# hello-robot/stretch_mujoco

Measured on AMD Instinct MI355X. Metric: env-steps/sec (whole node), 4096 parallel Stretch envs in total, higher is better.
Workload: dtype f32

## Files before the change

__graft_entry__.py:

```python
import os
import subprocess
import sys

ROOT = os.path.dirname(os.path.abspath(__file__))
sys.path.insert(0, ROOT)


def build() -> None:
    env = dict(os.environ)
    subprocess.check_call(["make", "-j6", "-C", os.path.join(ROOT, "stretch_mujoco_amd", "csrc")], env=env)
    subprocess.check_call(["make", "-C", os.path.join(ROOT, "oracle")], env=env)
    subprocess.check_call(["make", "-j4", "-C", os.path.join(ROOT, "tests", "emul")], env=env)
    subprocess.check_call(["make", "-j2", "-C", os.path.join(ROOT, "tests", "emul_contacts")], env=env)
    subprocess.check_call(["make", "-C", os.path.join(ROOT, "tests", "rccl_stub")], env=env)
    import stretch_mujoco_amd
    from stretch_mujoco_amd import lib

    L = lib.load()
    for sym in lib.EXPORTS:
        getattr(L, sym)


def smoke() -> None:
    import numpy as np
    import torch

    from oracle.oracle import Oracle
    from stretch_mujoco_amd import StretchBatchSimulator

    B, settle, nsteps = 8, 300, 100
    ctrl = np.array([2, -1, 0.6, 0.1, 1, -0.4, 0.5, 0.02, 0.3, -0.2], np.float32)
    o = Oracle(open(os.path.join(ROOT, "stretch_mujoco_amd", "models", "stretch_empty.smjb"), "rb").read())
    o.set_option("solver", 2)
    o.arr("ctrl")[:] = ctrl
    o.step(settle)
    sim = StretchBatchSimulator(num_envs=B, device="cuda:0", solver="newton")
    sim.start(home=False)
    dev = sim.device
    sim.ctrl[:] = torch.tensor(ctrl, device=dev).unsqueeze(1)
    sim.qpos[:] = torch.tensor(o.arr("qpos"), dtype=torch.float32, device=dev).unsqueeze(1)
    sim.qvel[:] = torch.tensor(o.arr("qvel"), dtype=torch.float32, device=dev).unsqueeze(1)
    sim.qacc_warmstart[:] = torch.tensor(o.arr("qacc_warmstart"), dtype=torch.float32, device=dev).unsqueeze(1)
    sim.step(nsteps)
    torch.cuda.synchronize()
    o.step(nsteps)
    qpos = sim.qpos.t().cpu().numpy()
    err = np.abs(qpos - o.arr("qpos")[None, :]).max()
    f = sim.info[3]
    flags = int(((f & 1).max() | (f & 2).max() | (f & 4).max() | (f & 8).max()).item())
    print(f"smoke: {B} envs x {nsteps} steps, max |qpos - oracle| = {err:.3e}, nefc = {int(sim.info[0, 0])}, flags = {flags}")
    assert np.isfinite(qpos).all(), "non-finite state"
    assert err < 1e-4, f"HIP path deviates from the fp64 oracle: {err}"
    assert flags == 0 and int(sim.nstep.min()) == int(sim.nstep.max()) == nsteps, "an env was flagged or ran fewer steps than asked"
    sim.stop()
    print(mujoco_status())


def mujoco_status() -> str:
    sys.path.insert(0, os.path.join(ROOT, "tools"))
    import mujoco_harness

    if not mujoco_harness.have_mujoco():
        return mujoco_harness.UNVERIFIED
    try:
        res = mujoco_harness.compare("stretch_empty", steps=1000)
        return res["verdict"] + " (tools/mujoco_harness.py; the HIP kernels are tested against that restatement)"
    except Exception as e:
        return f"mujoco is importable but the Appendix-D harness failed ({type(e).__name__}: {e}); MuJoCo parity UNVERIFIED"


if __name__ == "__main__":
    build()
    if len(sys.argv) > 1 and sys.argv[1] == "smoke":
        smoke()
```

stretch_mujoco_amd/csrc/smj_model.h:

```cpp
#pragma once
#include <stdint.h>

#if defined(SMJ_SAT)
#define NSAT SMJ_SAT
#define NVP 32
#ifndef SMJ_SAT_ROWS
#define SMJ_SAT_ROWS 320
#define SMJ_SAT_CONTACTS 64
#define SMJ_SAT_DENSE 256
#endif
#define NEFC SMJ_SAT_ROWS
#define NCON SMJ_SAT_CONTACTS
#define NDR SMJ_SAT_DENSE
#ifndef SMJ_SAT_EXT
#define SMJ_SAT_EXT 4
#endif
#ifndef SMJ_SAT_PGS
#define SMJ_SAT_PGS (SMJ_SAT_DENSE < 160 ? SMJ_SAT_DENSE : 160)
#endif
#define NXS SMJ_SAT_EXT
static_assert(NDR % 16 == 0 && NDR <= NEFC, "dense rows: whole 16-row blocks (matT_J, MFMA k-steps)");
#define NENT 5
#elif defined(SMJ_BIG)
#define NVP 64
#ifndef SMJ_NVS
#define SMJ_NVS 64
#endif
#define NVS SMJ_NVS
#if SMJ_NVS == 64
#define NEFC 224
#define NCON 64
#elif defined(SMJ_BIG_ROWS)
#define NEFC SMJ_BIG_ROWS
#define NCON SMJ_BIG_CONTACTS
#else
#define NEFC 160
#define NCON 48
#endif
#define NENT 8
#elif defined(SMJ_TALL)
#define NVP 32
#ifdef SMJ_TALL_ROWS
#define NEFC SMJ_TALL_ROWS
#define NCON SMJ_TALL_CONTACTS
#else
#define NEFC 160
#define NCON 48
#endif
#define NENT 5
#else
#define NVP 32
#define NEFC 80
#define NCON 16
#define NENT 5
#endif
#ifndef NVS
#define NVS NVP
#endif
#ifndef NSAT
#define NSAT 0
#endif
#ifndef NDR
#define NDR NEFC
#endif
static_assert(NVS % 2 == 0 && NVS <= NVP && (NVP == 64 ? NVS >= 38 : NVS == NVP), "column capacity: even (packed pairs), odd row stride NVS + 1");
#define NBP 32
#define NBT (NBP + NSAT)
#define NCG 128

#define SMJ_MODEL_I32(X)                                                                                          \
  X(body_parentid) X(k_body_jump) X(body_rootid) X(body_jntadr) X(body_jntnum) X(body_dofadr) X(body_dofnum) X(k_body_level)     \
  X(k_body_subtreesize) X(k_body_dofmask_lo) X(k_body_dofmask_hi) X(k_root_list) X(k_gc_body)                     \
  X(jnt_type) X(jnt_qposadr) X(jnt_dofadr) X(jnt_bodyid) X(jnt_limited)                                           \
  X(dof_bodyid) X(dof_jntid) X(dof_parentid) X(k_dof_anc_adr) X(k_dof_anc_num) X(k_dof_anc) X(k_dof_velmask_lo)   \
  X(k_dof_velmask_hi) X(k_dof_qposadr) X(k_ldl_i) X(k_ldl_j) X(k_ldl_lact) X(k_fric_dof) X(k_limit_jnt) X(k_act_dof) X(k_dof_act)                         \
  X(geom_type) X(geom_bodyid) X(geom_hulladr) X(geom_hullnum)                                                     \
  X(site_bodyid)                                                                           \
  X(eq_obj1id) X(eq_obj2id) X(eq_active)                                                                          \
  X(actuator_trntype) X(actuator_trnid) X(actuator_ctrllimited) X(actuator_forcelimited) X(actuator_biastype)     \
  X(pair_geom1) X(pair_geom2) X(pair_condim) X(k_planepair) X(k_cgeom) X(k_convpair) X(k_convpair_s1) X(k_convpair_s2) X(k_convpair_ss)

#define SMJ_MODEL_F32(X)                                                                                          \
  X(body_pos) X(body_quat) X(k_body_inertia_local) X(body_gcmass) X(body_gcipos) X(body_subtreemass)              \
  X(jnt_pos) X(jnt_axis) X(jnt_stiffness) X(jnt_range) X(jnt_margin) X(jnt_solref) X(jnt_solimp) X(qpos0)         \
  X(qpos_spring)                                                                                                  \
  X(dof_armature) X(dof_damping) X(dof_frictionloss) X(dof_invweight0) X(dof_solref) X(dof_solimp)                \
  X(geom_pos) X(k_geom_mat) X(geom_size) X(geom_rbound) X(k_geom_bcenter) X(geom_rgba) X(geom_invweight0)         \
  X(k_hull_vert4) X(geom_aabb) X(geom_ccenter) X(k_convpair_rsum) X(k_cgeom_half) X(k_cgeom_lcen)                                                                             \
  X(site_pos) X(k_site_mat)                                                                                       \
  X(eq_data) X(eq_solref) X(eq_solimp)                                                                            \
  X(actuator_gear) X(actuator_gainprm) X(actuator_biasprm) X(actuator_ctrlrange) X(actuator_forcerange)           \
  X(k_act_moment) X(key_ctrl) X(k_ldl_damp) X(k_ldl_dcoef) X(k_ldl_lcoef) X(k_act_mom) X(k_dof_actmom)                                                                                     \
  X(pair_friction) X(pair_solref) X(pair_solimp) X(pair_margin) X(pair_gap)

struct DevModel {
  int nq, nv, nu, nbody, njnt, ngeom, nsite, neq, npair, nlevel, nfric, nlimit, nplanepair, nldl, nlidar, imu_site,
      ngc, nroot, nkey, ncgeom, nconvpair, njump, maxsubtree;
  int iterations, warmstart, pgs_fixed_iter, max_con_pair, solver , ls_iterations, convex_pairs;
  float grad_noise;
  int pgs_island_stop;
  int qcqp_exact;
  int pgs_dual_ws;
  int sep_cache;
  int manifold_cache;
  int multi_serial;
  int pgs_cap;
  int row_limit;
  int multiccd;
  float ls_tolerance;
  float timestep, gravity[3], impratio, tolerance, meaninertia, lidar_cutoff;
  int nsat, nq_all, nv_all, nbody_all, nfric_main, nlimit_main;
  const int* k_satrec;
  int nsgeom, nstatpair, grid_dim[3];
  float grid_org[3], grid_h, grid_margin;
  const int* k_sgrec;
  const int* k_sprec;
  const int* k_spair;
  const int* k_grid_adr;
  const int* k_grid_list;
  const int* k_sg_cell;
  const float* k_sg_bound;
  const float* k_sgw;
#define X(n) const int* n;
  SMJ_MODEL_I32(X)
#undef X
#define X(n) const float* n;
  SMJ_MODEL_F32(X)
#undef X
  const int* k_lanerec;
  const int* k_pprec;
  const int* k_cgrec;
  const int* k_rowrec;
  const int* k_cprec;
};
enum { SMJ_CP_PAIR = 0, SMJ_CP_G1, SMJ_CP_G2, SMJ_CP_S1, SMJ_CP_S2, SMJ_CP_MARGIN, SMJ_CP_MG, SMJ_CP_CONDIM, SMJ_CP_FRIC = 8, SMJ_CP_SOLIMP = 13,
       SMJ_CP_SOLREF = 18, SMJ_CP_RBMIN = 20 ,
       SMJ_CP_B1 = 21, SMJ_CP_B2 = 22 , SMJ_CP_STRIDE = 24 };
enum { SMJ_RR_TYPE = 0, SMJ_RR_ID, SMJ_RR_D1, SMJ_RR_D2, SMJ_RR_Q1, SMJ_RR_Q2, SMJ_RR_V1, SMJ_RR_V2, SMJ_RR_DATA = 8, SMJ_RR_DIAG = 13,
       SMJ_RR_FLOSS = 14, SMJ_RR_SOLREF = 15, SMJ_RR_SOLIMP = 17, SMJ_RR_SAT = 22 , SMJ_RR_SDOF = 23 , SMJ_RR_STRIDE = 24 };
constexpr int smj_lr_act(int nent) { return 76 + ((7 * nent + 3) & ~3); }
constexpr int smj_lr_stride(int nent) { return smj_lr_act(nent) + 28; }
enum { SMJ_LR_KIN = 0, SMJ_LR_BODY = 36, SMJ_LR_DOF = 60, SMJ_LR_ENT = 76, SMJ_LR_ACT = smj_lr_act(NENT), SMJ_LR_STRIDE = smj_lr_stride(NENT) };
enum { SMJ_PP_PAIR = 0, SMJ_PP_G1, SMJ_PP_G2, SMJ_PP_B1, SMJ_PP_B2, SMJ_PP_T2, SMJ_PP_MARGIN, SMJ_PP_RBOUND2, SMJ_PP_BCEN2 = 8,
       SMJ_PP_POS1 = 11, SMJ_PP_MAT1 = 14, SMJ_PP_POS2 = 23, SMJ_PP_MAT2 = 26, SMJ_PP_SIZE2 = 35, SMJ_PP_CONDIM = 38, SMJ_PP_MG = 39,
       SMJ_PP_FRIC = 40, SMJ_PP_SOLIMP = 45, SMJ_PP_SOLREF = 50, SMJ_PP_BOX2 = 52 ,
       SMJ_PP_STRIDE = 60 };
enum { SMJ_CG_GEOM = 0, SMJ_CG_BODY, SMJ_CG_META, SMJ_CG_POS = 3, SMJ_CG_MAT = 6, SMJ_CG_LCEN = 15, SMJ_CG_HALF = 18, SMJ_CG_CCEN = 21,
       SMJ_CG_SIZE = 24, SMJ_CG_RBOUND = 27, SMJ_CG_STRIDE = 28 };

enum { SMJ_SR_BODY = 0, SMJ_SR_JTYPE, SMJ_SR_QADR, SMJ_SR_DADR, SMJ_SR_NDOF, SMJ_SR_JNT, SMJ_SR_F = 8,
       SMJ_SR_POS = SMJ_SR_F + 0, SMJ_SR_QUAT = SMJ_SR_F + 3, SMJ_SR_JPOS = SMJ_SR_F + 7, SMJ_SR_JAXIS = SMJ_SR_F + 10, SMJ_SR_Q0 = SMJ_SR_F + 13,
       SMJ_SR_INL = SMJ_SR_F + 14, SMJ_SR_ARM = SMJ_SR_F + 24, SMJ_SR_DAMP = SMJ_SR_F + 30, SMJ_SR_STIFF = SMJ_SR_F + 36, SMJ_SR_SPRING = SMJ_SR_F + 37,
       SMJ_SR_GCMASS = SMJ_SR_F + 38, SMJ_SR_GCIPOS = SMJ_SR_F + 39, SMJ_SR_STRIDE = 52 };
struct SmjStageLayout {
  int qpos, qvel, warm, ctrl, bctl, nstep, info, actlen, actvel, base, gyro, accel, xpose, stride;
};
constexpr SmjStageLayout smj_stage_layout(int nvp, int nbp, int nsat = 0) {
  SmjStageLayout L{};
  L.qpos = 0; L.qvel = L.qpos + nvp + 8 + 7 * nsat; L.warm = L.qvel + nvp + 6 * nsat; L.ctrl = L.warm + nvp + 6 * nsat; L.bctl = L.ctrl + 16; L.nstep = L.bctl + 8;
  L.info = L.nstep + 4; L.actlen = L.info + 4; L.actvel = L.actlen + 16; L.base = L.actvel + 16; L.gyro = L.base + 4;
  L.accel = L.gyro + 4; L.xpose = L.accel + 4; L.stride = L.xpose + 12 * nbp;
  return L;
}
struct DevState {
  int B;
  long ld;
  float* qpos;
  float* qvel;
  float* ctrl;
  float* warm;
  int* nstep;
  float* act_len;
  float* act_vel;
  float* base;
  float* gyro;
  float* accel;
  float* lidar;
  int* info;
  float* debug;
  float* prof;
  float* xpose;
  float* bctl;
  float* stage;
  SmjStageLayout lay;
  const int* order;
  int* cost;
  int* redo;
  int redo_worker;
// ... 68 lines not shown
```

stretch_mujoco_amd/csrc/smj_model_load.h:

```cpp
#pragma once
#include <stdint.h>
#include <stdio.h>
#include <math.h>
#include <string.h>

#include <map>
#include <string>
#include <vector>

#include "smj_model.h"

struct SmjBlobEntry {
  char name[48];
  uint32_t dtype, ndim, shape[4];
  uint64_t offset, nbytes;
};

struct SmjBlob {
  const uint8_t* p;
  size_t n;
  bool valid() const {
    if (!p || n < 16) return false;
    uint32_t cnt;
    memcpy(&cnt, p + 8, 4);
// ... 177 lines not shown
    int* k = rec.data() + (size_t)(nstat + L) * SMJ_RR_STRIDE;
    const int j = gi("k_limit_jnt", L >> 1), d = gi("jnt_dofadr", j);
    k[SMJ_RR_SAT] = sat_of(d, &k[SMJ_RR_SDOF]);
    k[SMJ_RR_TYPE] = 3; k[SMJ_RR_ID] = j; k[SMJ_RR_D1] = d; k[SMJ_RR_D2] = (L & 1) ? 1 : -1; k[SMJ_RR_Q1] = gi("jnt_qposadr", j);
    k[SMJ_RR_V1] = fb(gf("jnt_range", 2 * j + (L & 1))); k[SMJ_RR_V2] = fb(gf("jnt_margin", j));
    k[SMJ_RR_DIAG] = fb(gf("dof_invweight0", d));
    k[SMJ_RR_SOLREF] = fb(gf("jnt_solref", 2 * j)); k[SMJ_RR_SOLREF + 1] = fb(gf("jnt_solref", 2 * j + 1));
    for (int q = 0; q < 5; q++) k[SMJ_RR_SOLIMP + q] = fb(gf("jnt_solimp", 5 * j + q));
  }
  return rec;
}

static inline std::vector<int> smj_build_cprec(const DevModel& m, std::map<std::string, std::vector<int>>& I,
                                               std::map<std::string, std::vector<float>>& F, bool stat = false) {
  const int np = stat ? m.nstatpair : m.nconvpair;
  std::vector<int> rec((size_t)(np > 0 ? np : 1) * SMJ_CP_STRIDE, 0);
  auto fb = [](float v) { int b; memcpy(&b, &v, 4); return b; };
  auto gi = [&](const char* nm, size_t k) { const std::vector<int>& v = I[nm]; return k < v.size() ? v[k] : 0; };
  auto gf = [&](const char* nm, size_t k) { const std::vector<float>& v = F[nm]; return k < v.size() ? v[k] : 0.f; };
  std::map<int, int> dslot, sslot;
  if (stat) {
    for (int c = 0; c < m.ncgeom; c++) dslot[gi("k_cgeom", c)] = c;
    for (int c = 0; c < m.nsgeom; c++) sslot[gi("k_sgeom", c)] = c;
  }
  for (int t = 0; t < np; t++) {
    int* k = rec.data() + (size_t)t * SMJ_CP_STRIDE;
    const int p = gi(stat ? "k_statpair" : "k_convpair", t);
    k[SMJ_CP_PAIR] = p; k[SMJ_CP_G1] = gi("pair_geom1", p); k[SMJ_CP_G2] = gi("pair_geom2", p);
    if (stat) {
      k[SMJ_CP_S1] = sslot.count(k[SMJ_CP_G1]) ? -1 - sslot[k[SMJ_CP_G1]] : dslot[k[SMJ_CP_G1]];
      k[SMJ_CP_S2] = sslot.count(k[SMJ_CP_G2]) ? -1 - sslot[k[SMJ_CP_G2]] : dslot[k[SMJ_CP_G2]];
    } else { k[SMJ_CP_S1] = gi("k_convpair_s1", t); k[SMJ_CP_S2] = gi("k_convpair_s2", t); }
    k[SMJ_CP_MARGIN] = fb(gf("pair_margin", p)); k[SMJ_CP_MG] = fb(gf("pair_margin", p) - gf("pair_gap", p)); k[SMJ_CP_CONDIM] = gi("pair_condim", p);
    for (int q = 0; q < 5; q++) { k[SMJ_CP_FRIC + q] = fb(gf("pair_friction", 5 * p + q)); k[SMJ_CP_SOLIMP + q] = fb(gf("pair_solimp", 5 * p + q)); }
    k[SMJ_CP_SOLREF] = fb(gf("pair_solref", 2 * p)); k[SMJ_CP_SOLREF + 1] = fb(gf("pair_solref", 2 * p + 1));
    const float r1 = gf("geom_rbound", k[SMJ_CP_G1]), r2 = gf("geom_rbound", k[SMJ_CP_G2]);
    k[SMJ_CP_RBMIN] = fb(r1 < r2 ? r1 : r2);
    k[SMJ_CP_B1] = gi("geom_bodyid", k[SMJ_CP_G1]); k[SMJ_CP_B2] = gi("geom_bodyid", k[SMJ_CP_G2]);
  }
  return rec;
}

template <class Up>
int smj_load_model(const void* blob, size_t nbytes, DevModel& m, Up& up, std::string& err, const SmjCaps* caps, int ncaps, int* chosen) {
  if (!blob || nbytes < 16 || memcmp(blob, "SMJB0001", 8) != 0) { err = "not an SMJB model blob"; return -1; }
  SmjBlob b{static_cast<const uint8_t*>(blob), nbytes};
  if (!b.valid()) { err = "model blob: truncated or corrupt entry table"; return -3; }
  auto geti = [&](const char* name, int idx, int* out) -> bool {
    const SmjBlobEntry* e = b.find(name);
    if (!e || e->dtype != 1 || e->nbytes < 4u * (idx + 1)) { err = std::string("model blob: missing int ") + name; return false; }
    memcpy(out, b.p + e->offset + 4 * idx, 4);
    return true;
  };
  auto getf = [&](const char* name, int idx, float* out) -> bool {
    const SmjBlobEntry* e = b.find(name);
    if (!e || e->dtype != 0 || e->nbytes < 8u * (idx + 1)) { err = std::string("model blob: missing scalar ") + name; return false; }
    double v;
    memcpy(&v, b.p + e->offset + 8 * idx, 8);
    *out = (float)v;
    return true;
  };
#define GI(field, name, idx) if (!geti(name, idx, &m.field)) return -3;
#define GF(field, name, idx) if (!getf(name, idx, &m.field)) return -3;
  GI(nq_all, "dims", 0) GI(nv_all, "dims", 1) GI(nu, "dims", 2) GI(nbody_all, "dims", 3) GI(njnt, "dims", 4) GI(ngeom, "dims", 5)
  m.nq = m.nq_all; m.nv = m.nv_all; m.nbody = m.nbody_all; m.nsat = 0;
  if (b.find("k_nsat")) {
    GI(nsat, "k_nsat", 0)
    if (m.nsat > 0) { GI(nq, "k_main_dims", 0) GI(nv, "k_main_dims", 1) GI(nbody, "k_main_dims", 2) GI(njnt, "k_main_dims", 3) }
  }
  GI(nsite, "dims", 6) GI(neq, "dims", 8) GI(nkey, "dims", 11) GI(npair, "dims", 12)
  GI(nlevel, "k_nlevel", 0) GI(nfric, "k_nfric", 0) GI(nlimit, "k_nlimit", 0) GI(nplanepair, "k_nplanepair", 0)
  GI(nldl, "k_nldl", 0) GI(imu_site, "sensor_imu_site", 0) GI(ngc, "k_ngc", 0) GI(nroot, "k_nroot", 0)
  GI(njump, "k_njump", 0) GI(maxsubtree, "k_maxsubtree", 0) GI(ncgeom, "k_ncgeom", 0) GI(nconvpair, "k_nconvpair", 0) GI(iterations, "opt_iterations", 0)
  GF(timestep, "opt_timestep", 0) GF(gravity[0], "opt_gravity", 0) GF(gravity[1], "opt_gravity", 1)
  GF(gravity[2], "opt_gravity", 2) GF(impratio, "opt_impratio", 0) GF(tolerance, "opt_tolerance", 0)
  GF(meaninertia, "stat_meaninertia", 0) GF(lidar_cutoff, "sensor_lidar_cutoff", 0)
#undef GI
#undef GF
  if (m.nsat > 0 && (m.ngeom >= 65536 || m.npair >= (1 << 19))) { err = "satellite builds: at most 65535 geoms and 524287 collision pairs (16-bit geom ids per contact, the PGS row key)"; return -4; }
  {
    const SmjBlobEntry* e = b.find("sensor_lidar_site");
    m.nlidar = e ? (int)(e->nbytes / 4) : 0;
  }
  m.row_limit = 0; m.pgs_cap = 0; m.warmstart = 1; m.pgs_fixed_iter = 0; m.qcqp_exact = 0; m.grad_noise = 4e-6f; m.pgs_island_stop = 1; m.pgs_dual_ws = 1; m.max_con_pair = 4; m.solver = 0; m.convex_pairs = 1; m.multiccd = 1; m.sep_cache = getenv("SMJ_NO_SEPCACHE") ? 0 : 1; m.manifold_cache = (getenv("SMJ_NO_MCACHE") || m.nv_all <= 32) ? 0 : 1;    m.multi_serial = 0; m.ls_iterations = 50; m.ls_tolerance = 0.01f;
  char buf[256];
  int pick = -1, first = 0;
  {
    const SmjBlobEntry* e = b.find("k_capacity_hint");
    int hint = 0;
    if (e && e->dtype == 1 && e->nbytes >= 4) memcpy(&hint, b.p + e->offset, 4);
    if (hint > 0 && ncaps > 1) first = 1;
  }
  for (int v = first; v < ncaps && pick < 0; v++)
    if ((m.nsat > 0) == (caps[v].nsat > 0) && m.nsat <= caps[v].nsat &&
        m.nv <= (caps[v].nvs ? caps[v].nvs : caps[v].nvp) && m.nbody <= caps[v].nbp && m.nq <= caps[v].nvp + 8 && m.nldl <= caps[v].nent * 64) pick = v;
  if (pick < 0 && first > 0)
    for (int v = 0; v < first && pick < 0; v++)
      if ((m.nsat > 0) == (caps[v].nsat > 0) && m.nsat <= caps[v].nsat &&
          m.nv <= (caps[v].nvs ? caps[v].nvs : caps[v].nvp) && m.nbody <= caps[v].nbp && m.nq <= caps[v].nvp + 8 && m.nldl <= caps[v].nent * 64) pick = v;
  if (pick < 0 || m.nu > 16) {
    const SmjCaps& c = caps[ncaps - 1];
    snprintf(buf, sizeof buf, "model exceeds kernel capacity (nv %d<=%d, nbody %d<=%d, nq %d<=%d, nu %d<=16, mass-matrix entries %d<=%d, satellites %d)",
             m.nv, c.nvp, m.nbody, c.nbp, m.nq, c.nvp + 8, m.nu, m.nldl, c.nent * 64, m.nsat);
    err = buf;
    return -4;
  }
  if (chosen) *chosen = pick;
  const int nent = caps[pick].nent;
  if (m.neq + m.nfric > 64) { err = "too many static constraint rows"; return -4; }
  if (2 * m.nlimit > 64) { err = "too many limited joints"; return -4; }
  if (m.ngc > 16) { err = "more than 16 gravity-compensated bodies"; return -4; }
  if (m.njump > 6) { err = "body tree deeper than 64 levels"; return -4; }
  if (m.ncgeom > NCG) { err = "too many geoms in non-plane collision pairs"; return -4; }
  if (m.nconvpair >= 65536) { err = "more than 65535 non-plane collision pairs (the survivor list holds 16-bit pair indices)"; return -4; }
  std::map<std::string, std::vector<int>> hosti;
  std::map<std::string, std::vector<float>> hostf;
#define X(n)                                                                               \
  {                                                                                        \
    const SmjBlobEntry* e = b.find(#n);                                                    \
    if (!e || e->dtype != 1) { err = "model blob: missing i32 array " #n; return -3; }     \
    std::vector<int> h(e->nbytes / 4 ? e->nbytes / 4 : 1, 0);                              \
    memcpy(h.data(), b.p + e->offset, e->nbytes);                                          \
    m.n = up.i32(h);                                                                       \
    hosti[#n] = h;                                                                         \
    if (!m.n) { err = "device allocation failed for " #n; return -2; }                     \
  }
  SMJ_MODEL_I32(X)
#undef X
#define X(n)                                                                               \
  {                                                                                        \
    const SmjBlobEntry* e = b.find(#n);                                                    \
    if (!e || e->dtype != 0) { err = "model blob: missing f64 array " #n; return -3; }     \
    size_t cnt = e->nbytes / 8;                                                            \
    std::vector<float> h(cnt ? cnt : 1, 0.f);                                              \
    const double* src = reinterpret_cast<const double*>(b.p + e->offset);                  \
    for (size_t i = 0; i < cnt; i++) h[i] = (float)src[i];                                 \
    m.n = up.f32(h);                                                                       \
    hostf[#n] = h;                                                                         \
    if (!m.n) { err = "device allocation failed for " #n; return -2; }                     \
  }
  SMJ_MODEL_F32(X)
#undef X
  m.nsgeom = 0; m.nstatpair = 0; m.k_sgrec = m.k_sprec = m.k_spair = m.k_grid_adr = m.k_grid_list = m.k_sg_cell = nullptr; m.k_sg_bound = nullptr; m.k_sgw = nullptr;
  if (b.find("k_nsgeom")) {
    if (!geti("k_nsgeom", 0, &m.nsgeom) || !geti("k_nstatpair", 0, &m.nstatpair)) return -3;
    if (m.nsgeom > 512) { err = "more than 512 static collision geoms (the static broadphase's candidate word holds 9 bits of static geom index)"; return -4; }
    if (m.nstatpair > 0 && m.nsat == 0) { err = "static collision pairs (k_statpair) without satellites: only the satellite builds run collision_static; rebuild the blob (model_fuse.prepare_for_kernels)"; return -4; }
    if (m.nsgeom > 0) {
      for (int q = 0; q < 3; q++) { if (!geti("k_grid", q, &m.grid_dim[q]) || !getf("k_grid_f", q, &m.grid_org[q])) return -3; }
      if (!getf("k_grid_f", 3, &m.grid_h) || !getf("k_grid_f", 4, &m.grid_margin)) return -3;
      auto loadi = [&](const char* name, const int** dst) -> bool {
        const SmjBlobEntry* e = b.find(name);
        if (!e || e->dtype != 1) { err = std::string("model blob: missing i32 array ") + name; return false; }
        std::vector<int> h(e->nbytes / 4 ? e->nbytes / 4 : 1, 0);
        memcpy(h.data(), b.p + e->offset, e->nbytes);
        hosti[name] = h;
        *dst = up.i32(h);
        return *dst != nullptr;
      };
      const int* dummy = nullptr;
      if (!loadi("k_sgeom", &dummy) || !loadi("k_statpair", &dummy) || !loadi("k_spair", &m.k_spair) || !loadi("k_grid_adr", &m.k_grid_adr) ||
          !loadi("k_grid_list", &m.k_grid_list) || !loadi("k_sg_cell", &m.k_sg_cell)) return err.empty() ? -2 : -3;
      {
        const SmjBlobEntry* e = b.find("geom_aabb");
        (void)e;
      }
      std::vector<int> sg = smj_build_cgrec(m, hosti, hostf, true), spr = smj_build_cprec(m, hosti, hostf, true);
// ... 75 lines not shown
```

stretch_mujoco_amd/csrc/smj_step_impl.h:

```cpp
#pragma once
#ifndef SMJ_PROFILING
#define SMJ_PROFILING 1
#endif
#include <cstddef>
#include "smj_model.h"
#include "smj_wave.h"
#include "smj_sat_mem.h"

#define JS (NVS + 1)
#define MS (NVS + 1)
#define SMJ_MINVAL 1e-15f
#define SMJ_MINIMP 0.0001f
#define SMJ_MAXIMP 0.9999f

enum { JT_FREE = 0, JT_BALL = 1, JT_SLIDE = 2, JT_HINGE = 3 };
enum { GT_PLANE = 0, GT_SPHERE = 2, GT_CAPSULE = 3, GT_ELLIPSOID = 4, GT_CYLINDER = 5, GT_BOX = 6, GT_MESH = 7 };
enum { CT_EQUALITY = 0, CT_FRICTION = 1, CT_LIMIT = 3, CT_CONTACT_FRICTIONLESS = 5, CT_CONTACT_ELLIPTIC = 7, CT_NONE = -1 };

#if NSAT > 0
#define NCGS (NCG + 1)
#define NSURV 128
#else
#define NCGS NCG
#endif
// ... 181 lines not shown
      }
    }
    if (bad) {
#pragma unroll
      for (int i = 0; i < N; i++) res[i] = 0;
      return 0;
    }
    float x[N], nn = 0;
#pragma unroll
    for (int i = 0; i < N; i++) {
      float sv = -b[i];
#pragma unroll
      for (int k = 0; k < i; k++) sv -= L[i * N + k] * x[k];
      x[i] = sv * Li[i];
    }
#pragma unroll
    for (int i = N - 1; i >= 0; i--) {
      float sv = x[i];
#pragma unroll
      for (int k = i + 1; k < N; k++) sv -= L[k * N + i] * x[k];
      x[i] = sv * Li[i];
    }
#pragma unroll
    for (int i = 0; i < N; i++) { res[i] = x[i]; nn += x[i] * x[i]; }
    const float val = nn - r2;
    if (val < vtol && (exact || la == 0.f || val > -vtol)) break;
    float q = 0;
#pragma unroll
    for (int i = 0; i < N; i++) {
      float sv = res[i];
#pragma unroll
      for (int k = 0; k < i; k++) sv -= L[i * N + k] * x[k];
      x[i] = sv * Li[i];
      q += x[i] * x[i];
    }
    float delta;
    if (exact) {
      delta = val * fast_rcp(2.f * q);
      if (delta < dtol) break;
    } else {
      const float nrm = nn * fast_rsqrt(nn);
      delta = (nrm - r) * nn * fast_rcp(r * q);
      if (fabsf(delta) < dtol + drel * la) break;
      if (fabsf(delta) < 3e-3f * (la + dmin)) {
        const float lan = fmaxf(0.f, la + delta), d = lan - la;
#pragma unroll
        for (int i = N - 1; i >= 0; i--) {
          float sv = x[i];
#pragma unroll
          for (int k = i + 1; k < N; k++) sv -= L[k * N + i] * x[k];
          x[i] = sv * Li[i];
        }
#pragma unroll
        for (int i = 0; i < N; i++) res[i] -= d * x[i];
        la = lan;
        break;
      }
    }
    la = fmaxf(0.f, la + delta);
  }
#pragma unroll
  for (int i = 0; i < N; i++) res[i] *= dd[i];
  la_io = la;
  return la != 0;
}

SMJ_DEV float impedance(const float* solimp, float pos, float margin) {
  float dmin = fminf(SMJ_MAXIMP, fmaxf(SMJ_MINIMP, solimp[0])), dmax = fminf(SMJ_MAXIMP, fmaxf(SMJ_MINIMP, solimp[1]));
  float width = fmaxf(SMJ_MINVAL, solimp[2]), mid = fminf(SMJ_MAXIMP, fmaxf(SMJ_MINIMP, solimp[3])), power = fmaxf(1.0f, solimp[4]);
  if (dmin == dmax) return 0.5f * (dmin + dmax);
  float x = fabsf(pos - margin) / width, y;
  if (x >= 1) return dmax;
  if (x <= 0) return dmin;
  if (power == 1.0f) y = x;
  else if (power == 2.0f) y = (x <= mid) ? x * x / mid : 1 - (1 - x) * (1 - x) / (1 - mid);
  else if (x <= mid) y = powf(x, power) / powf(mid, power - 1);
  else y = 1 - powf(1 - x, power) / powf(1 - mid, power - 1);
  return dmin + y * (dmax - dmin);
}

#ifdef SMJ_EMUL
static long smj_emul_sep_skips = 0;
static long smj_emul_ext_steps = 0;
static long smj_emul_mc_hits = 0;
static long smj_emul_isl_total = 0, smj_emul_isl_swept = 0;
#endif
struct StepKernel {
  const DevModel& M;
  const DevState& S;
  Smem& s;
  int env;

  PL<float[6]> cdof, cdof_dot;
  PL<float> qvel_r, g_r, qacc_r;
  PL<float> f_r[NPS], r_r[NPS], ARinv_r[NPS];
  PL<float> qla_r;
  int nefc, ncon, niter, flags;
  float* ppc = nullptr;
  int step_base = 0;
  int pipe_chunk = 0;
  bool parked = false;
  bool split_on = false, rev = false;
  bool serial_redo = false;

  SMJ_DEV StepKernel(const DevModel& M_, const DevState& S_, Smem& s_, int env_) : M(M_), S(S_), s(s_), env(env_) {}

  SMJ_DEV static uint64_t mk64(int lo, int hi) { return (uint64_t)(uint32_t)lo | ((uint64_t)(uint32_t)hi << 32); }

  struct KinTab {
    PL<int> parent, level;
    PL<int[6]> jump;
    PL<float[3]> pos;
    PL<float[4]> quat;
    PL<int[2]> jtype, jqadr, jdadr;
    PL<float[2]> jq0;
    PL<float[6]> jaxis, jpos;
  };
  SMJ_DEV const int* lanerec(int ol, int off) const {
    return static_cast<const int*>(__builtin_assume_aligned(M.k_lanerec + ol * SMJ_LR_STRIDE + off, 16));
  }
  SMJ_DEV static float asf(int b) { return __builtin_bit_cast(float, b); }
  SMJ_DEV void load(KinTab& t) {
    LANES {
      const int* r = lanerec(opaque(lane), SMJ_LR_KIN);
      int v[35];
      for (int k = 0; k < 35; k++) v[k] = r[k];
      t.parent[lane] = v[0]; t.level[lane] = v[1];
      for (int q = 0; q < 6; q++) t.jump[lane][q] = v[2 + q];
      for (int k = 0; k < 3; k++) t.pos[lane][k] = asf(v[8 + k]);
      for (int k = 0; k < 4; k++) t.quat[lane][k] = asf(v[11 + k]);
      for (int u = 0; u < 2; u++) {
        t.jtype[lane][u] = v[15 + u]; t.jqadr[lane][u] = v[17 + u]; t.jdadr[lane][u] = v[19 + u]; t.jq0[lane][u] = asf(v[21 + u]);
      }
      for (int k = 0; k < 6; k++) { t.jaxis[lane][k] = asf(v[23 + k]); t.jpos[lane][k] = asf(v[29 + k]); }
    }
  }
  struct BodyTab {
    PL<int> root, subsize, parent, dofadr, dofnum;
    PL<int[6]> jump;
    PL<uint64_t> dofmask;
    PL<float[10]> inl;
  };
  SMJ_DEV void load(BodyTab& t) {
    LANES {
      const int* r = lanerec(opaque(lane), SMJ_LR_BODY);
      int v[23];
      for (int k = 0; k < 23; k++) v[k] = r[k];
      t.root[lane] = v[0]; t.subsize[lane] = v[1]; t.parent[lane] = v[2]; t.dofadr[lane] = v[3]; t.dofnum[lane] = v[4];
      for (int q = 0; q < 6; q++) t.jump[lane][q] = v[5 + q];
      t.dofmask[lane] = mk64(v[11], v[12]);
      for (int k = 0; k < 10; k++) t.inl[lane][k] = asf(v[13 + k]);
    }
  }
  struct DofTab {
    PL<int> body, jtype, qadr, first, bsub;
    PL<uint64_t> velmask;
    PL<float> damp, stiff, spring;
    PL<int[2]> act;
    PL<float[2]> actmom;
  };
  SMJ_DEV void load(DofTab& t) {
    LANES {
      const int* r = lanerec(opaque(lane), SMJ_LR_DOF);
      int v[14];
      for (int k = 0; k < 14; k++) v[k] = r[k];
      t.body[lane] = v[0]; t.jtype[lane] = v[1]; t.qadr[lane] = v[2]; t.first[lane] = v[3]; t.bsub[lane] = v[4];
      t.velmask[lane] = mk64(v[5], v[6]);
      t.damp[lane] = asf(v[7]); t.stiff[lane] = asf(v[8]); t.spring[lane] = asf(v[9]);
      for (int u = 0; u < 2; u++) { t.act[lane][u] = v[10 + u]; t.actmom[lane][u] = asf(v[12 + u]); }
    }
  }
  struct EntryTab {
    PL<int[NENT]> i, j, lact;
    PL<float[NENT]> arm, damp, dcoef, lcoef;
  };
  SMJ_DEV void load(EntryTab& t, bool implicit) {
    LANES {
      const int* r = lanerec(opaque(lane), SMJ_LR_ENT);
      for (int u = 0; u < NENT; u++) { t.i[lane][u] = r[u]; t.j[lane][u] = r[NENT + u]; t.arm[lane][u] = asf(r[2 * NENT + u]); }
      if (implicit)
        for (int u = 0; u < NENT; u++) {
          t.lact[lane][u] = r[3 * NENT + u]; t.damp[lane][u] = asf(r[4 * NENT + u]); t.dcoef[lane][u] = asf(r[5 * NENT + u]);
          t.lcoef[lane][u] = asf(r[6 * NENT + u]);
        }
    }
  }
  struct ActTab {
    PL<int[4]> dof, qadr;
    PL<float[4]> mom;
    PL<float[8]> prm;
    PL<int> flags;
    PL<int> gc_body, gc_mlo, gc_mhi;
    PL<float> gc_mass, gc_x, gc_y, gc_z;
  };
  SMJ_DEV void load(ActTab& t) {
    LANES {
      const int* r = lanerec(opaque(lane), SMJ_LR_ACT);
      int v[28];
      for (int k = 0; k < 28; k++) v[k] = r[k];
      for (int u = 0; u < 4; u++) { t.dof[lane][u] = v[u]; t.qadr[lane][u] = v[4 + u]; t.mom[lane][u] = asf(v[8 + u]); }
      for (int k = 0; k < 8; k++) t.prm[lane][k] = asf(v[12 + k]);
      t.flags[lane] = v[20]; t.gc_body[lane] = v[21]; t.gc_mlo[lane] = v[22]; t.gc_mhi[lane] = v[23];
      t.gc_mass[lane] = asf(v[24]); t.gc_x[lane] = asf(v[25]); t.gc_y[lane] = asf(v[26]); t.gc_z[lane] = asf(v[27]);
    }
// ... 3310 lines not shown
  SMJ_DEV void gj_solve_lds(PL<float>& x) {
    const int n = M.nv;
    LANES { if (lane < NVS) s.u.n.H[lane][NVS] = lane < n ? x[lane] : 0.f; }
    SYNC();
    for (int k = 0; k < n; k++) {
      const float rp = fast_rcp(fmaxf(uni(s.u.n.H[k][k]), 1e-30f));
      LANES {
        if (lane < n && lane != k) {
          float* row = s.u.n.H[lane];
          const float* piv = s.u.n.H[k];
          const float mult = row[k] * rp;
          int j = k + 1;
          for (; j + 8 <= n; j += 8) {
            float a[8], b[8];
#pragma unroll
            for (int u = 0; u < 8; u++) { a[u] = row[j + u]; b[u] = piv[j + u]; }
#pragma unroll
            for (int u = 0; u < 8; u++) row[j + u] = a[u] - mult * b[u];
          }
          for (; j < n; j++) row[j] -= mult * piv[j];
          row[NVS] -= mult * piv[NVS];
        }
      }
      SYNC();
    }
    LANES { x[lane] = lane < n ? s.u.n.H[lane][NVS] * fast_rcp(fmaxf(s.u.n.H[lane][lane], 1e-30f)) : 0.f; }
    SYNC();
  }
  SMJ_DEV void solve_H(PL<float>& x, bool rare = false) {
#if NVP == 32
    if (M.nv <= 26) gj_solve<26>(x);
    else gj_solve<NVP>(x);
#else
    if (rare || M.nv > 50) gj_solve_lds(x);
#if NVS >= 50
    else if (M.nv > 38) gj_solve<50>(x);
#endif
    else gj_solve<38>(x);
#endif
  }

  SMJ_DEV float ls_eval(NRow& nr0, const float* qg, float a, float& d1, float& d2) {
    const int ne = nefc;
    PL<float> p0, p1, p2;
    LANES { p0[lane] = 0.f; p1[lane] = 0.f; p2[lane] = 0.f; }
    ROWS_BEGIN(rb, ne) LANES {
      float c0 = 0, c1 = 0, c2 = 0;
      if (lane + rb < ne) {
        const int t = nr.type[lane];
        const float x = nr.jar[lane] + a * nr.jv[lane];
        if (t == CT_EQUALITY) { c0 = nr.q0[lane]; c1 = nr.q1[lane]; c2 = nr.q2[lane]; }
        else if (t == CT_FRICTION) {
          const float fl = nr.fl[lane], rf = nr.R[lane] * fl;
          if (x <= -rf) { c0 = fl * (-0.5f * rf - nr.jar[lane]); c1 = -fl * nr.jv[lane]; }
          else if (x >= rf) { c0 = fl * (-0.5f * rf + nr.jar[lane]); c1 = fl * nr.jv[lane]; }
          else { c0 = nr.q0[lane]; c1 = nr.q1[lane]; c2 = nr.q2[lane]; }
        } else if (t == CT_LIMIT || t == CT_CONTACT_FRICTIONLESS) {
          if (x < 0) { c0 = nr.q0[lane]; c1 = nr.q1[lane]; c2 = nr.q2[lane]; }
        } else if (nr.c0[lane] >= 0) {
          const float* k = nr.cq[lane];
          const float mu = k[6], Dm = k[5], N = k[0] + a * k[1], Tsq = k[2] + a * (2 * k[3] + a * k[4]);
          if (Tsq <= 0) { if (N < 0) { c0 = nr.q0[lane]; c1 = nr.q1[lane]; c2 = nr.q2[lane]; } }
          else {
            const float Ti = fast_rsqrt(Tsq), T = Tsq * Ti;
            if (N >= mu * T) {}
            else if (mu * N + T <= 0) { c0 = nr.q0[lane]; c1 = nr.q1[lane]; c2 = nr.q2[lane]; }
            else {
              const float w = k[3] + a * k[4], N1 = k[1], T1 = w * Ti, T2 = k[4] * Ti - w * w * Ti * Ti * Ti;
              const float NT = N - mu * T, NT1 = N1 - mu * T1;
              const float v = 0.5f * Dm * NT * NT, g = Dm * NT * NT1, h = Dm * (NT1 * NT1 - NT * mu * T2);
              c2 = 0.5f * h; c1 = g - h * a; c0 = v - a * g + 0.5f * h * a * a;
            }
          }
        }
      }
      p0[lane] += c0; p1[lane] += c1; p2[lane] += c2;
    } ROWS_END_RO()
    const float q0 = qg[0] + wave_sum(p0), q1 = qg[1] + wave_sum(p1), q2 = qg[2] + wave_sum(p2);
    d1 = 2 * a * q2 + q1;
    d2 = 2 * q2;
    return a * a * q2 + a * q1 + q0;
  }

  SMJ_DEV void solve_newton(bool dbg, float* pc, long long& t0, bool prof) {
#define TICK(slot) if (prof) { const long long t1 = smj_clock(); pc[slot] += (float)(t1 - t0); t0 = t1; }
    const int nv = M.nv, ne = nefc;
    NRow nr0;
    PL<float> qacc, Ma, Mv, grad, search, tmpv;
    if (ne == 0) {
      build_dense(false);
      LANES { qacc[lane] = lane < nv ? g_r[lane] : 0.f; }
      solve_H(qacc, true);
      LANES {
        qacc_r[lane] = lane < nv ? qacc[lane] : 0.f;
        if (lane < nv) { s.qacc[lane] = qacc[lane]; s.warm[lane] = qacc[lane]; s.tmp[lane] = g_r[lane]; }
#if NSAT > 0
        if (lane >= 32 && lane - 32 < M.nsat) {
          const int si = lane - 32;
          float A[21], x[6];
          for (int k = 0; k < 21; k++) A[k] = s.sat.Mb[si][k];
          for (int k = 0; k < 6; k++) { x[k] = s.sat.x[SX_G][si][k]; s.sat.x[SX_TMP][si][k] = x[k]; }
          sat_solve6(A, x);
          for (int k = 0; k < 6; k++) s.sat.x[SX_QA][si][k] = k < s.sat.ndof[si] ? x[k] : 0.f;
        }
#endif
      }
      niter = 0;
      SYNC();
      return;
    }
    ROWS_BEGIN_(rb, ne, false) LANES {
      const int row = lane + rb;
      float vel = 0;
      const bool on = row < ne;
      if (on) {
        const float* jr = jrow(row);
        for (int k = 0; k < nv; k++) vel += jr[k] * s.qvel[k];
#if NSAT > 0
        vel += sat_jdot(row, SX_V);
#endif
      }
      nr.type[lane] = on ? s.etype[row] : CT_NONE;
      nr.R[lane] = on ? s.eR[row] : 1.f;
      nr.D[lane] = on ? 1.0f / s.eR[row] : 0.f;
      nr.fl[lane] = on ? s.efloss[row] : 0.f;
      nr.aref[lane] = on ? -s.eBv[row] * vel - s.eK[row] * s.eimp[row] * (s.epos[row] - s.emargin[row]) : 0.f;
      int c0 = -1;
      if (on && s.etype[row] == CT_CONTACT_ELLIPTIC && s.cefc[s.eid[row]] == row) c0 = s.eid[row];
      nr.c0[lane] = c0;
      nr.state[lane] = 0; nr.jar[lane] = 0.f; nr.jv[lane] = 0.f; nr.force[lane] = 0.f; nr.q0[lane] = 0.f; nr.q1[lane] = 0.f; nr.q2[lane] = 0.f;
      for (int k = 0; k < 7; k++) nr.cq[lane][k] = 0.f;
      if (c0 >= 0) {
        const float mu = contact_mu(c0);
        nr.cq[lane][6] = mu;
        nr.cq[lane][5] = (1.0f / s.eR[row]) / fmaxf(mu * mu * (1 + mu * mu), SMJ_MINVAL);
      }
      if (dbg && row < NEFC) s.earef[row] = nr.aref[lane];
    } ROWS_END_RW(rb)
#if NSAT > 0
    const int nvt = M.nv_all;
#else
    const int nvt = nv;
#endif
    const float scale = 1.0f / (M.meaninertia * (float)(nvt > 1 ? nvt : 1));
    LANES { qacc[lane] = (lane < nv && M.warmstart) ? s.warm[lane] : 0.f; }
    mat_M(Ma, qacc);
#if NSAT > 0
    if (!M.warmstart) { LANES { if (lane >= 32 && lane - 32 < M.nsat) for (int k = 0; k < 6; k++) s.sat.x[SX_QA][lane - 32][k] = 0.f; } }
    sat_matM(SX_MA, SX_QA);
    SYNC();
#endif
    ROWS_BEGIN(rb, ne) mat_J_exact(nr.jar, qacc, nr.aref, rb); ROWS_END_RW(rb)
    float cost = 0;
    TICK(SMJ_PROF_WARM)
    int iter = 0;
    bool at_update = false;
    for (; iter < M.iterations;) {
      TICK(SMJ_PROF_PGS)
      cost = newton_update(nr0, true);
      float gauss;
      {
        PL<float> gs;
        LANES {
          gs[lane] = lane < nv ? qacc[lane] * (0.5f * Ma[lane] - g_r[lane]) : 0.f;
#if NSAT > 0
          if (lane >= 32 && lane - 32 < M.nsat)
// ... 23 lines not shown
            g2[lane] += gr * gr;
            gsig[lane] |= fabsf(gr) > M.grad_noise * (fabsf(ma) + fabsf(gg) + fabsf(jf));
          }
        }
#endif
      }
      const float gnorm = sqrtf(wave_sum(g2));
      if (iter > 0 && (scale * gnorm < M.tolerance || wave_ballot(gsig) == 0)) { at_update = true; break; }
      TICK(SMJ_PROF_N_GRAD)
      ROWS_BEGIN(rb, ne) LANES {
        const int row = lane + rb;
        if (row < NEFC) s.ediag[row] = (row < ne && nr.state[lane] == 1) ? nr.D[lane] : 0.f;
      } ROWS_END_RO()
      uint64_t conemask;
      {
        PL<int> cz;
#if NSAT > 0
        SYNC();
#endif
        LANES {
          int z = 0;
          if (lane < ncon) {
            const int r0 = s.cefc[lane];
            z = r0 >= 0 && s.cdim[lane] >= 3 && s.estate[r0 >= 0 ? r0 : 0] == 4;
#if NSAT > 0
            if (z && s.sat.chs[lane] < 0) {
              for (int j = 0; j < s.cdim[lane]; j++) s.ediag[r0 + j] = 1.0f / s.eR[r0 + j];
              z = 0;
            }
#endif
          }
          cz[lane] = z;
        }
        conemask = wave_ballot(cz);
      }
      SYNC();
      TICK(SMJ_PROF_N_XA)
#if SMJ_W2_NEWTON
      fork2(W2_SAT_NEWTON, (int)(uint32_t)conemask, (int)(uint32_t)(conemask >> 32));
#endif
      {
        constexpr int NT = (NVS + 15) / 16, NTRI = NT * (NT + 1) / 2, KB = NVP == 32 ? 16 : 8;
        const int ksteps = (ndense() + 3) >> 2;
        PL<F4v> acc[NTRI];
        LANES {
#pragma unroll
          for (int t = 0; t < NTRI; t++)
            for (int r = 0; r < 4; r++) acc[t][lane].r[r] = 0.f;
        }
#pragma unroll
        for (int kb = 0; kb < NDR / 4; kb += KB) {
          if (kb < 16 ? kb < ksteps : __builtin_expect(kb < ksteps, 0)) {
            PL<float[KB]> b[NT], wk;
            LANES {
#pragma unroll
              for (int ks = 0; ks < KB; ks++) {
                const int k = 4 * (kb + ks) + (lane >> 4), c = lane & 15;
                if (kb + ks < NDR / 4) {
                  wk[lane][ks] = s.ediag[k];
#pragma unroll
                  for (int t = 0; t < NT; t++) b[t][lane][ks] = s.J[k][16 * t + c];
                }
              }
            }
#pragma unroll
            for (int ks = 0; ks < KB; ks++) {
              if (kb + ks < ksteps && kb + ks < NDR / 4) {
                PL<float> pa[NT], pb[NT];
                LANES {
#pragma unroll
                  for (int t = 0; t < NT; t++) { pb[t][lane] = b[t][lane][ks]; pa[t][lane] = wk[lane][ks] * pb[t][lane]; }
                }
#pragma unroll
                for (int ta = 0; ta < NT; ta++)
#pragma unroll
                  for (int tb = 0; tb <= ta; tb++) mfma16x16x4(acc[ta * (ta + 1) / 2 + tb], pa[ta], pb[tb]);
              }
            }
          }
        }
        long long th = 0;
        if (prof) { th = smj_clock(); pc[SMJ_PROF_H_K] += (float)(th - t0); }
        int nks = 0;
        for (uint64_t cm = conemask; cm;) {
          const int c = ffs64(cm);
          cm &= cm - 1;
          const int r0 = uni(s.cefc[c]), dim = uni(s.cdim[c]);
          if (r0 >= ndense()) continue;
          for (int q0 = 0; q0 < dim; q0 += 4) {
            nks++;
            PL<float> pa[NT], pb[NT];
            LANES {
              const int q = q0 + (lane >> 4), col = lane & 15, qc = q < 6 ? q : 5;
              const float on = q < dim ? 1.f : 0.f;
              float hq[6];
#if NSAT > 0
              const int hc = s.sat.chs[c];
#else
              const int hc = c;
#endif
#pragma unroll
              for (int p = 0; p < 6; p++) hq[p] = on * s.u.n.cH[hc][6 * qc + p];
#pragma unroll
              for (int t = 0; t < NT; t++) {
                float jv[6], av = 0.f;
#pragma unroll
                for (int p = 0; p < 6; p++) jv[p] = s.J[r0 + p < NDR ? r0 + p : NDR - 1][16 * t + col];
#pragma unroll
                for (int p = 0; p < 6; p++) av += hq[p] * jv[p];
                pa[t][lane] = av;
                pb[t][lane] = on * s.J[r0 + qc < NDR ? r0 + qc : NDR - 1][16 * t + col];
              }
            }
#pragma unroll
            for (int ta = 0; ta < NT; ta++)
#pragma unroll
              for (int tb = 0; tb <= ta; tb++) mfma16x16x4(acc[ta * (ta + 1) / 2 + tb], pa[ta], pb[tb]);
          }
        }
        if (prof) { const long long t1 = smj_clock(); pc[SMJ_PROF_H_CONE] += (float)(t1 - th); th = t1; pc[SMJ_PROF_H_NKS] += (float)nks; }
        LANES {
#pragma unroll
          for (int ta = 0; ta < NT; ta++)
#pragma unroll
            for (int tb = 0; tb <= ta; tb++) {
#pragma unroll
              for (int r = 0; r < 4; r++) {
                const int row = 16 * ta + (lane >> 4) * 4 + r, col = 16 * tb + (lane & 15);
                if (NVS % 16 == 0 || (row < NVS && col < NVS)) {
                  float v = acc[ta * (ta + 1) / 2 + tb][lane].r[r];
                  v += s.MM[row][col];
                  s.u.n.H[row][col] = v;
                  if (ta != tb) s.u.n.H[col][row] = v;
                }
              }
            }
        }
      }
      SYNC();
      if (prof) pc[SMJ_PROF_H_STORE] += (float)(smj_clock() - t0);
      TICK(SMJ_PROF_N_HMFMA)
      LANES { search[lane] = lane < nv ? grad[lane] : 0.f; }
#if NSAT > 0
      const long long tsh = prof ? smj_clock() : 0;
#if SMJ_W2_NEWTON
      WG_BARRIER();
#else
      sat_hessian(conemask);
      SYNC();
#endif
      if (prof) pc[SMJ_PROF_SAT_H] += (float)(smj_clock() - tsh);
      if (next_sat > 0) {
        sat_extend_hessian(next_sat, conemask);
        LANES {
          if (lane >= NVS && lane < NVS + 6 * next_sat) { const int e = (lane - NVS) / 6; search[lane] = s.sat.x[SX_GRAD][s.sat.xs[e]][lane - NVS - 6 * e]; }
        }
        solve_ext_schur(search, next_sat);
        LANES {
          if (lane >= NVS && lane < NVS + 6 * next_sat) { const int e = (lane - NVS) / 6; s.sat.x[SX_SRCH][s.sat.xs[e]][lane - NVS - 6 * e] = -search[lane]; }
        }
      } else solve_H(search);
#if !SMJ_W2_NEWTON
      sat_solve_own();
#endif
      SYNC();
#else
      solve_H(search);
#endif
      TICK(SMJ_PROF_N_FACTSOLVE)
      PL<float> sq;
      LANES {
        search[lane] = lane < nv ? -search[lane] : 0.f; sq[lane] = search[lane] * search[lane];
#if NSAT > 0
        if (lane >= 32 && lane - 32 < M.nsat)
          for (int k = 0; k < 6; k++) sq[lane] += s.sat.x[SX_SRCH][lane - 32][k] * s.sat.x[SX_SRCH][lane - 32][k];
#endif
      }
      const float snorm = sqrtf(wave_sum(sq));
      TICK(SMJ_PROF_N_SOLVE)
      mat_M(Mv, search);
#if NSAT > 0
      sat_matM(SX_MV, SX_SRCH);
      SYNC();
      ROWS_BEGIN(rb, ne) {
        mat_J(nr.jv, search, rb);
        LANES { if (lane + rb < ne) nr.jv[lane] += sat_jdot(lane + rb, SX_SRCH); }
      } ROWS_END_RW(rb)
#else
      ROWS_BEGIN(rb, ne) mat_J(nr.jv, search, rb); ROWS_END_RW(rb)
#endif
      float qg[3];
      {
        PL<float> a1, a2;
        LANES {
          a1[lane] = lane < nv ? search[lane] * (Ma[lane] - g_r[lane]) : 0.f;
          a2[lane] = lane < nv ? 0.5f * search[lane] * Mv[lane] : 0.f;
#if NSAT > 0
          if (lane >= 32 && lane - 32 < M.nsat) {
            const int si = lane - 32;
            for (int k = 0; k < 6; k++) {
// ... 435 lines not shown
```

Baseline: 12.99 million.

## Batch cone Hessian k-steps via ballot-compacted descriptor list in groups of four

Replaces the serial per-cone loop that builds the cone-zone Hessian contributions. The new code first compacts all active cones into a list of k-step descriptors in shared scratch using a wave ballot and prefix popcount. It then loads the operands for four k-steps at once before issuing their MFMAs, with a scheduling barrier between the two phases, so the shared-memory loads can overlap. This adds register pressure, a sync, and padding work when the k-step count is not a multiple of four; the old serial path is kept for the emulator behind a flag.

```diff
diff --git a/__graft_entry__.py b/__graft_entry__.py
--- a/__graft_entry__.py
+++ b/__graft_entry__.py
@@ -12,6 +12,7 @@
     subprocess.check_call(["make", "-C", os.path.join(ROOT, "oracle")], env=env)
     subprocess.check_call(["make", "-j4", "-C", os.path.join(ROOT, "tests", "emul")], env=env)
     subprocess.check_call(["make", "-j2", "-C", os.path.join(ROOT, "tests", "emul_contacts")], env=env)
+    subprocess.check_call(["make", "-j2", "-C", os.path.join(ROOT, "tests", "emul_paths")], env=env)
     subprocess.check_call(["make", "-C", os.path.join(ROOT, "tests", "rccl_stub")], env=env)
     import stretch_mujoco_amd
     from stretch_mujoco_amd import lib
diff --git a/stretch_mujoco_amd/csrc/smj_model.h b/stretch_mujoco_amd/csrc/smj_model.h
--- a/stretch_mujoco_amd/csrc/smj_model.h
+++ b/stretch_mujoco_amd/csrc/smj_model.h
@@ -104,6 +104,7 @@
   int sep_cache;
   int manifold_cache;
   int multi_serial;
+  int cone_serial;
   int pgs_cap;
   int row_limit;
   int multiccd;
diff --git a/stretch_mujoco_amd/csrc/smj_model_load.h b/stretch_mujoco_amd/csrc/smj_model_load.h
--- a/stretch_mujoco_amd/csrc/smj_model_load.h
+++ b/stretch_mujoco_amd/csrc/smj_model_load.h
@@ -283,7 +283,7 @@
     const SmjBlobEntry* e = b.find("sensor_lidar_site");
     m.nlidar = e ? (int)(e->nbytes / 4) : 0;
   }
-  m.row_limit = 0; m.pgs_cap = 0; m.warmstart = 1; m.pgs_fixed_iter = 0; m.qcqp_exact = 0; m.grad_noise = 4e-6f; m.pgs_island_stop = 1; m.pgs_dual_ws = 1; m.max_con_pair = 4; m.solver = 0; m.convex_pairs = 1; m.multiccd = 1; m.sep_cache = getenv("SMJ_NO_SEPCACHE") ? 0 : 1; m.manifold_cache = (getenv("SMJ_NO_MCACHE") || m.nv_all <= 32) ? 0 : 1;    m.multi_serial = 0; m.ls_iterations = 50; m.ls_tolerance = 0.01f;
+  m.row_limit = 0; m.pgs_cap = 0; m.warmstart = 1; m.pgs_fixed_iter = 0; m.qcqp_exact = 0; m.grad_noise = 4e-6f; m.pgs_island_stop = 1; m.pgs_dual_ws = 1; m.max_con_pair = 4; m.solver = 0; m.convex_pairs = 1; m.multiccd = 1; m.sep_cache = getenv("SMJ_NO_SEPCACHE") ? 0 : 1; m.manifold_cache = (getenv("SMJ_NO_MCACHE") || m.nv_all <= 32) ? 0 : 1;    m.multi_serial = 0; m.cone_serial = 0; m.ls_iterations = 50; m.ls_tolerance = 0.01f;
   char buf[256];
   int pick = -1, first = 0;
   {
diff --git a/stretch_mujoco_amd/csrc/smj_step_impl.h b/stretch_mujoco_amd/csrc/smj_step_impl.h
--- a/stretch_mujoco_amd/csrc/smj_step_impl.h
+++ b/stretch_mujoco_amd/csrc/smj_step_impl.h
@@ -287,6 +287,7 @@
 #ifdef SMJ_EMUL
 static long smj_emul_sep_skips = 0;
 static long smj_emul_ext_steps = 0;
+static long smj_emul_cone_multi = 0;
 static long smj_emul_mc_hits = 0;
 static long smj_emul_isl_total = 0, smj_emul_isl_swept = 0;
 #endif
@@ -325,6 +326,7 @@
     return static_cast<const int*>(__builtin_assume_aligned(M.k_lanerec + ol * SMJ_LR_STRIDE + off, 16));
   }
   SMJ_DEV static float asf(int b) { return __builtin_bit_cast(float, b); }
+  SMJ_DEV static int fbits(float f) { return __builtin_bit_cast(int, f); }
   SMJ_DEV void load(KinTab& t) {
     LANES {
       const int* r = lanerec(opaque(lane), SMJ_LR_KIN);
@@ -3801,6 +3803,51 @@
     return a * a * q2 + a * q1 + q0;
   }
 
+  template <int NT>
+  SMJ_DEV void cone_operands(int lane, int r0, int dim, int q0, int hc, PL<float>* pa, PL<float>* pb) {
+#pragma clang fp contract(off)
+    const int q = q0 + (lane >> 4), col = lane & 15, qc = q < 6 ? q : 5;
+    const float on = q < dim ? 1.f : 0.f;
+    float hq[6];
+#pragma unroll
+    for (int p = 0; p < 6; p++) hq[p] = on * s.u.n.cH[hc][6 * qc + p];
+#pragma unroll
+    for (int t = 0; t < NT; t++) {
+      float jv[6], av = 0.f;
+#pragma unroll
+      for (int p = 0; p < 6; p++) jv[p] = s.J[r0 + p < NDR ? r0 + p : NDR - 1][16 * t + col];
+#pragma unroll
+      for (int p = 0; p < 6; p++) av += hq[p] * jv[p];
+      pa[t][lane] = av;
+      pb[t][lane] = on * s.J[r0 + qc < NDR ? r0 + qc : NDR - 1][16 * t + col];
+    }
+  }
+#ifdef SMJ_EMUL
+  template <int NT, int NTRI>
+  int cone_ksteps_serial(uint64_t conemask, PL<F4v> (&acc)[NTRI]) {
+    int nks = 0;
+    for (uint64_t cm = conemask; cm;) {
+      const int c = ffs64(cm);
+      cm &= cm - 1;
+      const int r0 = uni(s.cefc[c]), dim = uni(s.cdim[c]);
+      if (r0 >= ndense()) continue;
+      for (int q0 = 0; q0 < dim; q0 += 4) {
+        nks++;
+        PL<float> pa[NT], pb[NT];
+#if NSAT > 0
+        const int hc = s.sat.chs[c];
+#else
+        const int hc = c;
+#endif
+        LANES { cone_operands<NT>(lane, r0, dim, q0, hc, pa, pb); }
+        for (int ta = 0; ta < NT; ta++)
+          for (int tb = 0; tb <= ta; tb++) mfma16x16x4(acc[ta * (ta + 1) / 2 + tb], pa[ta], pb[tb]);
+      }
+    }
+    return nks;
+  }
+#endif
+
   SMJ_DEV void solve_newton(bool dbg, float* pc, long long& t0, bool prof) {
 #define TICK(slot) if (prof) { const long long t1 = smj_clock(); pc[slot] += (float)(t1 - t0); t0 = t1; }
     const int nv = M.nv, ne = nefc;
@@ -3990,40 +4037,62 @@
         long long th = 0;
         if (prof) { th = smj_clock(); pc[SMJ_PROF_H_K] += (float)(th - t0); }
         int nks = 0;
-        for (uint64_t cm = conemask; cm;) {
-          const int c = ffs64(cm);
-          cm &= cm - 1;
-          const int r0 = uni(s.cefc[c]), dim = uni(s.cdim[c]);
-          if (r0 >= ndense()) continue;
-          for (int q0 = 0; q0 < dim; q0 += 4) {
-            nks++;
-            PL<float> pa[NT], pb[NT];
+#ifdef SMJ_EMUL
+        if (M.cone_serial) nks = cone_ksteps_serial<NT, NTRI>(conemask, acc);
+        else
+#endif
+        if (conemask) {
+          constexpr int CB = 4;
+          static_assert(2 * NCON + CB <= NEFC && NCON <= 64 && NEFC < 4096, "the k-step list of the cone zone lives in s.eb");
+          PL<int> n1, n2, desc;
+          LANES {
+            int n = 0, d = 0;
+            if (lane < NCON && ((conemask >> lane) & 1)) {
+              const int r0 = s.cefc[lane], dim = s.cdim[lane];
+#if NSAT > 0
+              const int hc = s.sat.chs[lane];
+#else
+              const int hc = lane;
+#endif
+              if (r0 < ndense()) { n = dim > 4 ? 2 : 1; d = r0 | dim << 12 | hc << 20; }
+            }
+            n1[lane] = n >= 1; n2[lane] = n == 2; desc[lane] = d;
+          }
+          const uint64_t m1 = wave_ballot(n1), m2 = wave_ballot(n2);
+          LANES {
+            const uint64_t below = (1ull << lane) - 1;
+            const int at = popc64(m1 & below) + popc64(m2 & below);
+            if (n1[lane]) s.eb[at] = asf(desc[lane]);
+            if (n2[lane]) s.eb[at + 1] = asf(desc[lane] | 4 << 16);
+          }
+          nks = popc64(m1) + popc64(m2);
+          SYNC();
+#ifdef SMJ_EMUL
+          if (popc64(m1) >= 2) smj_emul_cone_multi++;
+#endif
+          for (int kb = 0; kb < nks; kb += CB) {
+            PL<float> pa[CB][NT], pb[CB][NT];
             LANES {
-              const int q = q0 + (lane >> 4), col = lane & 15, qc = q < 6 ? q : 5;
-              const float on = q < dim ? 1.f : 0.f;
-              float hq[6];
-#if NSAT > 0
-              const int hc = s.sat.chs[c];
-#else
-              const int hc = c;
-#endif
-#pragma unroll
-              for (int p = 0; p < 6; p++) hq[p] = on * s.u.n.cH[hc][6 * qc + p];
-#pragma unroll
-              for (int t = 0; t < NT; t++) {
-                float jv[6], av = 0.f;
-#pragma unroll
-                for (int p = 0; p < 6; p++) jv[p] = s.J[r0 + p < NDR ? r0 + p : NDR - 1][16 * t + col];
-#pragma unroll
-                for (int p = 0; p < 6; p++) av += hq[p] * jv[p];
-                pa[t][lane] = av;
-                pb[t][lane] = on * s.J[r0 + qc < NDR ? r0 + qc : NDR - 1][16 * t + col];
+              int d[CB];
+#pragma unroll
+              for (int j = 0; j < CB; j++) d[j] = fbits(s.eb[kb + j]);
+#pragma unroll
+              for (int j = 0; j < CB; j++) d[j] = opaque(kb + j < nks ? d[j] : d[0]);
+#pragma unroll
+              for (int j = 0; j < CB; j++) cone_operands<NT>(lane, d[j] & 4095, (d[j] >> 12) & 15, (d[j] >> 16) & 15, d[j] >> 20, pa[j], pb[j]);
+            }
+#ifndef SMJ_EMUL
+            __builtin_amdgcn_sched_barrier(0);
+#endif
+#pragma unroll
+            for (int j = 0; j < CB; j++) {
+              if (kb + j < nks) {
+#pragma unroll
+                for (int ta = 0; ta < NT; ta++)
+#pragma unroll
+                  for (int tb = 0; tb <= ta; tb++) mfma16x16x4(acc[ta * (ta + 1) / 2 + tb], pa[j][ta], pb[j][tb]);
               }
             }
-#pragma unroll
-            for (int ta = 0; ta < NT; ta++)
-#pragma unroll
-              for (int tb = 0; tb <= ta; tb++) mfma16x16x4(acc[ta * (ta + 1) / 2 + tb], pa[ta], pb[tb]);
           }
         }
         if (prof) { const long long t1 = smj_clock(); pc[SMJ_PROF_H_CONE] += (float)(t1 - th); th = t1; pc[SMJ_PROF_H_NKS] += (float)nks; }
```

New measurement: 13.00 million (median of 4 runs). Within noise of the previous version (+0.1%).
